# mikostrzewa/AprilSLAM

Hardware: AMD Instinct MI355X
Metric: frames/sec at 1280x720, 20 tags/frame (detection + batched PnP) (higher is better)
Workload: dtype u8/f64

## Files before the change

### aprilslam_amd/csrc/aprilslam.hip

```cpp
#include "../../include/aprilslam.h"

#include <algorithm>
#include <chrono>
#include <cmath>
#include <cstdarg>
#include <cstdio>
#include <cstring>
#include <memory>
#include <string>
#include <type_traits>
#include <vector>

#include "asl_common.h"
#include "tag_standard41h12.inc"
#include "k_wave.inc"

#include "k_threshold.inc"
#include "k_blur.inc"
#include "k_cc.inc"
#include "k_cluster.inc"
#include "k_seg.inc"
#include "k_quad.inc"
#include "k_decode.inc"
#include "k_pnp.inc"
// ... 472 lines not shown
    if (g.f == 2) {
        const unsigned int ntile = (unsigned int)(g.tw * g.th);
        const unsigned int nrest = (unsigned int)(g.sw - 4 * g.tw) * (unsigned int)g.sh + (unsigned int)(g.sh - 4 * g.th) * (unsigned int)(4 * g.tw);
        if (ntile)
            hipLaunchKernelGGL((g.channels == 1 ? k_decimate2_tiles<1> : k_decimate2_tiles<3>), dim3((ntile + 255) / 256, B), dim3(256), 0, st, d_frames, g,
                               d->dgray.p, d->tmin.p, d->tmax.p);
        if (nrest)
            hipLaunchKernelGGL((g.channels == 1 ? k_decimate_rest<1> : k_decimate_rest<3>), dim3((nrest + 255) / 256, B), dim3(256), 0, st, d_frames, g,
                               d->dgray.p);
    } else
        hipLaunchKernelGGL((g.channels == 1 ? k_decimate_minmax<1> : k_decimate_minmax<3>), dim3((g.sw + 63) / 64, (thx + 3) / 4, B), blk, 0, st, d_frames, g, d->dgray.p, d->tmin.p, d->tmax.p);

    d->qgray = d->dgray.p;
    if (d->blur.r) {
        STAGE("k_quad_blur");
        hipLaunchKernelGGL(k_quad_blur, dim3((g.sw + BLUR_TW - 1) / BLUR_TW, (g.sh + BLUR_TH - 1) / BLUR_TH, B), dim3(256), 0, st, d->dgray.p, g, d->blur,
                           d->bgray.p, d->tmin.p, d->tmax.p);
        d->qgray = d->bgray.p;
    }

    const int nwx = seg_nwx(g), pty = seg_point_tiles_y(g);
    const size_t nwords = (size_t)B * g.sh * nwx;
    STAGE("k_tile_cut");
    if (g.tw > 0 && g.th > 0)
        hipLaunchKernelGGL(k_tile_cut, dim3((((g.tw + 3) / 4) * ((g.th + 3) / 4) + 255) / 256, B), dim3(256), 0, st, d->tmin.p, d->tmax.p, g, d->tcut.p);
    STAGE("k_seg_tile");
    {
        const int ntiles = nwx * ((g.sh + SEG_TH - 1) / SEG_TH);
        hipLaunchKernelGGL(k_seg_tile, dim3((ntiles + SEG_TILE_WAVES - 1) / SEG_TILE_WAVES, 1, B), dim3(64 * SEG_TILE_WAVES), 0, st, d->qgray, d->tcut.p, g, nwx, ntiles,
                           d->wmask.p, d->bmask.p, d->parent.p, d->sizes.p, d->rootmask.p, d->seg_edges.p, d->dense_seg.p, d->counters.p);
        hipLaunchKernelGGL(k_seg_tile_dense, dim3(1024), dim3(64), 0, st, g, nwx, ntiles, d->wmask.p, d->bmask.p, d->parent.p, d->sizes.p,
                           d->rootmask.p, d->dense_seg.p, d->counters.p);
    }
    STAGE("k_seg_border");
    {
        const size_t nseams = nwx > 1 ? (size_t)B * g.sh * (nwx - 1) : 0;
        const unsigned int ncol_blocks = (unsigned int)((nseams + 63) / 64);
        const int nrb = (g.sh - 1) / SEG_TH;
        const unsigned int nrow_blocks = (unsigned int)nwx * (unsigned int)nrb * (unsigned int)B;
        if (ncol_blocks + nrow_blocks > 0)
            hipLaunchKernelGGL(k_seg_border, dim3(ncol_blocks + nrow_blocks), dim3(64), 0, st, d->wmask.p, d->bmask.p, d->seg_edges.p,
                               nwx * ((g.sh + SEG_TH - 1) / SEG_TH), g, nwx, d->parent.p, d->counters.p, ncol_blocks, nrb > 0 ? nrb : 1);
    }
    STAGE("k_seg_roots");
    hipLaunchKernelGGL(k_seg_roots, dim3((unsigned int)((nwords + 255) / 256)), dim3(256), 0, st, d->rootmask.p, g, nwx, d->parent.p, d->sizes.p);

    STAGE("k_seg_points");
    hipLaunchKernelGGL((k_seg_points<SEGP_PCAP, SEGP_RUNCAP, SEGP_NW, 1>), dim3(B, (nwx + SEGP_NW - 1) / SEGP_NW, pty), dim3(64 * SEGP_NW), 0, st,
                       d->wmask.p, d->bmask.p, g, nwx, d->parent.p, d->sizes.p, d->hkeys.p, d->hcounts.p, d->nslots - 1, d->stage_rec.p,
                       d->stage_pos.p, d->frame_cursor.p, d->stage_cap, d->dense_tiles.p, pty, d->counters.p);
    hipLaunchKernelGGL((k_seg_points<SEGP_PCAP_DENSE, SEGP_RUNCAP_DENSE, 1, 2>), dim3(256), dim3(64), 0, st, d->wmask.p, d->bmask.p, g, nwx,
                       d->parent.p, d->sizes.p, d->hkeys.p, d->hcounts.p, d->nslots - 1, d->stage_rec.p, d->stage_pos.p, d->frame_cursor.p,
                       d->stage_cap, d->dense_tiles.p, pty, d->counters.p);
    STAGE("k_cluster_filter");
    hipLaunchKernelGGL(k_cluster_filter, dim3((d->nslots + 1023) / 1024), dim3(1024), 0, st, d->hkeys.p, d->hcounts.p, d->nslots, g,
                       d->clusters.p, d->slot_cluster.p, d->class_lists.p, d->max_clusters, d->max_points, d->counters.p);
    STAGE("k_point_place");
    hipLaunchKernelGGL(k_point_place, dim3(16, B), dim3(256), 0, st, d->stage_rec.p, d->stage_pos.p, d->frame_cursor.p, d->stage_cap,
                       d->slot_cluster.p, d->points.p, d->counters.p);

    range_pop();
    range_push("S5 quad fit");
    for (int cls = 0; cls < NCLASSES; cls++) {
        static const char *const kFitStage[NCLASSES] = {"k_fit_quads<0>", "k_fit_quads<1>", "k_fit_quads<2>", "k_fit_quads<3>", "k_fit_quads<4>"};
        STAGE(kFitStage[cls]);
        launch_fit_class(d, g, cls, B, st);
    }

    STAGE("k_quad_finish");
    launch_quad_finish(d, g, st);
    range_pop();
    range_push("S6-S7 edge refinement, homography, decode");
    STAGE("k_quad_compact");
    hipLaunchKernelGGL(k_quad_compact, dim3((d->max_clusters + 1023) / 1024), dim3(1024), 0, st, d->quads.p, d->counters.p, d->max_clusters,
                       d->quad_list.p);
    unsigned int dgrid = std::min<unsigned int>(d->max_clusters, std::max<unsigned int>(8192u, 64u * B));
    STAGE("k_refine");
    hipLaunchKernelGGL((g.channels == 1 ? k_refine<1> : k_refine<3>), dim3(dgrid), dim3(64), 0, st, d->quads.p, d->counters.p, d->max_clusters, d_frames, g,
                       d->fam.reversed_border ? 1 : 0, d->refine, d->quadH.p, d->quad_list.p, d->side_mom.p);
    STAGE("k_homography");
    hipLaunchKernelGGL(k_homography, dim3(std::min<unsigned int>((d->max_clusters + 31) / 32, 2048u)), dim3(256), 0, st, d->quadH.p, d->counters.p, d->max_clusters,
                       d->quad_list.p, d->side_mom.p);
    STAGE("k_decode");
    hipLaunchKernelGGL((g.channels == 1 ? k_decode<1> : k_decode<3>), dim3(dgrid), dim3(64), 0, st, d->quads.p, d->quadH.p, d->counters.p, d->max_clusters, d_frames, g, d->fam,
                       d->maxhamming, d->dets.p, d->max_dets, d->counters.p, d->quad_list.p);

    range_pop();
    range_push("S9 PnP, S8 de-duplication");
    if (cam) {
        STAGE("k_pnp_dets");
        const int tpw = pnp_tpw(d->nd_guess ? d->nd_guess : (size_t)20 * B);
        hipLaunchKernelGGL(k_pnp_dets, dim3((d->max_dets + tpw - 1) / tpw), dim3(64), 0, st, d->dets.p, d->counters.p, d->max_dets, *cam, tpw);
    }
    STAGE("k_det_dedup");
    launch_dedup(S8Buffers{d->dets.p, d->counters.p, d->max_dets, d->frame_ndets.p, d->frame_idx.p, d->dets_per_frame, d->frame_nkeep.p, d->frame_off.p,
                           d->out_det.p, d->out_pose.p},
                 B, cam ? 1 : 0, st);
    range_pop();
    if (d->profiling && d->nev <= MAX_STAGES) HIPCHK(hipEventRecord(d->ev[d->nev], st));
    HIPCHK(hipGetLastError());
    return ASL_OK;
}

static CamDev make_cam(const asl_detector *d, const double *K, const double *dist, int n_dist, double tag_size)
{
    CamDev c;
    c.both_minima = d->pnp_both_minima; c.pad = 0;
    c.fx = K[0]; c.fy = K[4]; c.cx = K[2]; c.cy = K[5];
    c.k1 = c.k2 = c.p1 = c.p2 = c.k3 = 0;
    if (dist && n_dist >= 4) { c.k1 = dist[0]; c.k2 = dist[1]; c.p1 = dist[2]; c.p2 = dist[3]; }
    if (dist && n_dist >= 5) c.k3 = dist[4];
    c.half = (double)(float)(tag_size / 2);
    return c;
}

using clk = std::chrono::steady_clock;
static float msf(clk::time_point a, clk::time_point b) { return std::chrono::duration<float, std::milli>(b - a).count(); }

static int ensure_host_out(asl_detector *d, size_t want, size_t nframes)
{
    HIPCHK(d->host_nkeep.ensure(nframes, hipHostMallocDefault));
    if (want <= d->host_cap()) return ASL_OK;
    d->host_det.release(); d->host_pose.release();
    want = std::max<size_t>(want * 2, 4096);
    HIPCHK(d->host_det.ensure(want, hipHostMallocNonCoherent));
    HIPCHK(d->host_pose.ensure(want, hipHostMallocNonCoherent));
    return ASL_OK;
}

static int submit_batch(asl_detector *d, const uint8_t *d_frames, const Geom &g, hipStream_t st, const CamDev *cam)
{
    if (d->pending) return fail(ASL_EINVAL, "a batch is already in flight on this detector: collect it first");
    int rc = ensure_workspace(d, g);
    if (rc) return rc;
    d->t_submit = clk::now();
    rc = enqueue_detect(d, d_frames, g, st, cam);
    if (rc) return rc;
    HIPCHK(d->pinned_counters.ensure(CNT__N, hipHostMallocDefault));
    HIPCHK(hipMemcpyAsync(d->pinned_counters.p, d->counters.p, sizeof(long long) * CNT__N, hipMemcpyDeviceToHost, st));
    d->prefetched = 0;
    rc = ensure_host_out(d, std::min<size_t>(d->nd_guess, d->max_dets), (size_t)g.nframes);
    if (rc) return rc;
    HIPCHK(hipMemcpyAsync(d->host_nkeep.p, d->frame_nkeep.p, sizeof(unsigned int) * (size_t)g.nframes, hipMemcpyDeviceToHost, st));
    if (d->nd_guess > 0) {
        size_t guess = std::min<size_t>(d->nd_guess, d->max_dets);
        HIPCHK(hipMemcpyAsync(d->host_det.p, d->out_det.p, guess * sizeof(DetOut), hipMemcpyDeviceToHost, st));
        if (cam) HIPCHK(hipMemcpyAsync(d->host_pose.p, d->out_pose.p, guess * sizeof(PoseOut), hipMemcpyDeviceToHost, st));
        d->prefetched = guess;
    }
    d->pending = true;
    d->p_frames = d_frames; d->p_geom = g; d->p_stream = st; d->p_has_cam = cam != nullptr;
    if (cam) d->p_cam = *cam;
    d->t_enqueued = clk::now();
    return ASL_OK;
}

static int collect_batch(asl_detector *d, asl_detection *out, asl_pose *poses, int max_out, int *n_per_frame, int *n_out)
{
    if (!d->pending) return fail(ASL_EINVAL, "no batch in flight on this detector");
    const Geom g = d->p_geom;
    hipStream_t st = d->p_stream;
    const CamDev *cam = d->p_has_cam ? &d->p_cam : nullptr;
    clk::time_point t0 = d->t_submit, t1 = d->t_enqueued, t2 = t1;
    for (int attempt = 0; attempt < 4; attempt++) {
        if (attempt > 0) {
            d->pending = false;
            d->nd_guess = 0;
            int rc = submit_batch(d, d->p_frames, g, st, cam);
// ... 405 lines not shown
```

### aprilslam_amd/csrc/k_decode.inc

```

#define DEC_PROBE_GROUP 11
#define DEC_MAX_PROBES 44

__device__ __forceinline__ void half_angle_normal_dev(double a, double b, double *nx, double *ny)
{
    double r = sqrt(a * a + b * b);
    if (r == 0) { *nx = 1; *ny = 0; return; }
    double c2 = a / r;
    if (c2 >= 0) {
        double c = sqrt((1 + c2) / 2);
        *nx = c;
        *ny = b / (2 * r * c);
    } else {
        double s = sqrt((1 - c2) / 2);
        if (b < 0) s = -s;
        *ny = s;
        *nx = b / (2 * r * s);
    }
}

__device__ __forceinline__ double grp8_max(double v)
{
    v = fmax(v, dpp_mov<QUAD_XOR1>(0.0, v));
    v = fmax(v, dpp_mov<QUAD_XOR2>(0.0, v));
// ... 19 lines not shown
    const unsigned int nq = nq64 > (long long)max_clusters ? max_clusters : (unsigned int)nq64;
    const int lane = threadIdx.x & 63, r = lane & 7;
    for (unsigned int q0 = blockIdx.x * 32u; q0 < nq; q0 += gridDim.x * 32u) {
        const unsigned int qi = q0 + (threadIdx.x >> 3);
        const bool live = qi < nq;
        const unsigned int ci = quad_list[live ? qi : 0];
        double *const rec = corners_H + 10 * (size_t)ci;
        const double state = live ? rec[9] : 0.0;
        const bool todo = state == 0.5 || state == 0.25;
        const int e = r & 3;
        double Pex = todo ? rec[2 * e] : 0.0, Pey = todo ? rec[2 * e + 1] : 0.0;
        if (__any(state == 0.25)) {
            const double *in = edge_mom + ((size_t)(state == 0.25 ? ci : 0) * 4 + e) * 6;
            const double Mx = in[0], My = in[1], Mxx = in[2], Mxy = in[3], Myy = in[4], Nn = in[5];
            const double Ex = Mx / Nn, Ey = My / Nn;
            const double Cxx = Mxx / Nn - Ex * Ex, Cxy = Mxy / Nn - Ex * Ey, Cyy = Myy / Nn - Ey * Ey;
            double nx, ny;
            half_angle_normal_dev(Cyy - Cxx, -2 * Cxy, &nx, &ny);
            const double n0 = dpp_mov<QUAD_ROT1>(0.0, Ex), n1 = dpp_mov<QUAD_ROT1>(0.0, Ey), n2 = dpp_mov<QUAD_ROT1>(0.0, nx), n3 = dpp_mov<QUAD_ROT1>(0.0, ny);
            const double A00 = ny, A01 = -n3;
            const double A10 = -nx, A11 = n2;
            const double B0 = -Ex + n0;
            const double B1 = -Ey + n1;
            const double det = A00 * A11 - A10 * A01;
            const bool moved = fabs(det) > 0.001;
            const double W00 = A11 / det, W01 = -A01 / det;
            const double L0 = W00 * B0 + W01 * B1;
            const double cx = Ex + L0 * A00, cy = Ey + L0 * A10;
            const double fx = dpp_mov<QUAD_ROT3>(0.0, cx), fy = dpp_mov<QUAD_ROT3>(0.0, cy);
            const bool fm = dpp_mov<QUAD_ROT3>(0, moved ? 1 : 0) != 0;
            if (state == 0.25 && fm) { Pex = fx; Pey = fy; }
        }
        const int i = r >> 1;
        const double x = (i == 1 || i == 2) ? 1.0 : -1.0, y = (i >= 2) ? 1.0 : -1.0;
        const double u = __shfl(Pex, (lane & ~7) + i), v = __shfl(Pey, (lane & ~7) + i);
        double a[9];
        if ((r & 1) == 0) { a[0] = x; a[1] = y; a[2] = 1; a[3] = 0; a[4] = 0; a[5] = 0; a[6] = -x * u; a[7] = -y * u; a[8] = u; }
        else { a[0] = 0; a[1] = 0; a[2] = 0; a[3] = x; a[4] = y; a[5] = 1; a[6] = -x * v; a[7] = -y * v; a[8] = v; }
        int pos = r;
        bool ok = true;
#pragma unroll
        for (int col = 0; col < 8; col++) {
            const double val = pos >= col ? fabs(a[col]) : -1.0;
            const double mx = grp8_max(val);
            if (mx < 1e-10) ok = false;
            const int pivpos = grp8_min(val == mx ? pos : 99);
            const bool is_piv = pos == pivpos;
            if (is_piv) pos = col;
            else if (pos == col) pos = pivpos;
            const int src = grp8_owner(is_piv, lane);
            double piv[9];
#pragma unroll
            for (int j = col; j < 9; j++) piv[j] = __shfl(a[j], src);
            if (pos > col) {
                const double f = a[col] / piv[col];
                a[col] = 0.0;
#pragma unroll
                for (int j = col + 1; j < 9; j++) a[j] = a[j] - f * piv[j];
            }
        }
        double xs[8], mine = 0;
#pragma unroll
        for (int col = 7; col >= 0; col--) {
            double sum = 0;
#pragma unroll
            for (int k = col + 1; k < 8; k++) sum += a[k] * xs[k];
            const double xc = (a[8] - sum) / a[col];
            xs[col] = __shfl(xc, grp8_owner(pos == col, lane));
            if (r == col) mine = xs[col];
        }
        const bool all_ok = (__ballot(ok) >> (lane & ~7) & 0xFFull) == 0xFFull;
        if (todo) {
            rec[r] = mine;
            if (r == 0) { rec[8] = 1.0; rec[9] = all_ok ? 1.0 : 0.0; }
        }
    }
}

__device__ __forceinline__ void hproject_dev(const double *H, double x, double y, double *ox, double *oy)
{
    double xx = H[0] * x + H[1] * y + H[2];
    double yy = H[3] * x + H[4] * y + H[5];
    double zz = H[6] * x + H[7] * y + H[8];
    *ox = xx / zz;
    *oy = yy / zz;
}

struct GrayModel { double A[9], B[3], C[3]; };

__device__ __forceinline__ void gm_add_dev(GrayModel &gm, double x, double y, double gray)
{
    gm.A[0] += x * x; gm.A[1] += x * y; gm.A[2] += x; gm.A[4] += y * y; gm.A[5] += y; gm.A[8] += 1;
    gm.B[0] += x * gray; gm.B[1] += y * gray; gm.B[2] += gray;
}

__device__ __forceinline__ void gm_solve_dev(GrayModel &gm)
{
    const double *A = gm.A, *B = gm.B;
    double L[9], M[9], t[3];
    L[0] = sqrt(A[0]); L[3] = A[1] / L[0]; L[6] = A[2] / L[0];
    L[4] = sqrt(A[4] - L[3] * L[3]); L[7] = (A[5] - L[3] * L[6]) / L[4];
    L[8] = sqrt(A[8] - L[6] * L[6] - L[7] * L[7]);
    M[0] = 1 / L[0]; M[3] = -L[3] * M[0] / L[4]; M[4] = 1 / L[4];
    M[6] = (-L[6] * M[0] - L[7] * M[3]) / L[8]; M[7] = -L[7] * M[4] / L[8]; M[8] = 1 / L[8];
    t[0] = M[0] * B[0]; t[1] = M[3] * B[0] + M[4] * B[1]; t[2] = M[6] * B[0] + M[7] * B[1] + M[8] * B[2];
    gm.C[0] = M[0] * t[0] + M[3] * t[1] + M[6] * t[2];
    gm.C[1] = M[4] * t[1] + M[7] * t[2];
    gm.C[2] = M[8] * t[2];
}

__device__ __forceinline__ double gm_interp_dev(const GrayModel &gm, double x, double y) { return gm.C[0] * x + gm.C[1] * y + gm.C[2]; }

template <int CH>
__device__ __forceinline__ double value_for_pixel_dev(const uint8_t *frame, const Geom &g, double px, double py)
{
    int x1 = (int)floor(px - 0.5), x2 = (int)ceil(px - 0.5);
    double x = px - 0.5 - x1;
    int y1 = (int)floor(py - 0.5), y2 = (int)ceil(py - 0.5);
    double y = py - 0.5 - y1;
    if (x1 < 0 || x2 >= g.w || y1 < 0 || y2 >= g.h) return -1;
    return gray_at<CH>(frame, g, x1, y1) * (1 - x) * (1 - y) + gray_at<CH>(frame, g, x2, y1) * x * (1 - y) +
           gray_at<CH>(frame, g, x1, y2) * (1 - x) * y + gray_at<CH>(frame, g, x2, y2) * x * y;
}

__device__ __forceinline__ unsigned long long rotate90_dev(unsigned long long w, int nbits)
{
    int p = nbits;
    unsigned long long l = 0;
    if (nbits % 4 == 1) { p = nbits - 1; l = 1; }
    w = ((w >> l) << (p / 4 + l)) | (w >> (3 * p / 4 + l) << l) | (w & l);
    w &= ((1ull << nbits) - 1ull);
    return w;
}

#define PIX_EPS 9.5367431640625e-07

template <int CH>
__global__ void __launch_bounds__(64) k_refine(const QuadRec *__restrict__ quads, const long long *__restrict__ counters,
                                               unsigned int max_clusters, const uint8_t *__restrict__ frames, Geom g, int fam_reversed,
                                               int refine, double *__restrict__ Hout ,
                                               const unsigned int *__restrict__ quad_list, double *__restrict__ edge_mom )
{
    __shared__ double s_bx[64], s_by[64];
    __shared__ int s_bvalid[64];
    __shared__ double s_P[4][2];
    __shared__ int s_soff[5];
    __shared__ short s_probe[DEC_MAX_PROBES][64];
    __shared__ double s_enx[4], s_eny[4];
    int lane = threadIdx.x;
    PHASE_DECL();
    if (batch_poisoned(counters)) return;
    long long nq64 = counters[CNT_NQUADS];
    unsigned int nq = nq64 > (long long)max_clusters ? max_clusters : (unsigned int)nq64;

    for (unsigned int qi = blockIdx.x; qi < nq; qi += gridDim.x) {
        __syncthreads();
        PHASE_INIT();
        const unsigned int ci = quad_list[qi];
        const QuadRec *qp = quads + ci;
        const int q_valid = qp->valid, q_reversed = qp->reversed_border;
        if (lane == 0) Hout[10 * (size_t)ci + 9] = 0.0;
        if (!q_valid) continue;
        if (fam_reversed != q_reversed) continue;
        int fr = (int)(qp->key >> 48);
        const uint8_t *frame = frames + (size_t)fr * g.frame_pitch;
        if (lane < 4) {
            double px = qp->p[lane][0], py = qp->p[lane][1];
            if (g.f > 1) { px = (px - 0.5) * g.f + 0.5; py = (py - 0.5) * g.f + 0.5; }
// ... 73 lines not shown
                                }
                            }
                            at_prev = at[DEC_PROBE_GROUP - 1];
                        }
                    } else
                    for (int j0 = 0; j0 < nprobe; j0 += DEC_PROBE_GROUP) {
                        unsigned int raw[DEC_PROBE_GROUP], shv[DEC_PROBE_GROUP];
                        bool inside[DEC_PROBE_GROUP];
#pragma unroll
                        for (int u = 0; u < DEC_PROBE_GROUP; u++) {
                            double t = -(range + 1) + 0.25 * (j0 + u);
                            int xi = (int)(x0 + t * nx + PIX_EPS), yi = (int)(y0 + t * ny + PIX_EPS);
                            inside[u] = j0 + u < nprobe && (unsigned int)xi < (unsigned int)g.w && (unsigned int)yi < (unsigned int)g.h;
                            raw[u] = pixel_fetch<CH>(frame, g, inside[u] ? xi : 0, inside[u] ? yi : 0, &shv[u]);
                        }
#pragma unroll
                        for (int u = 0; u < DEC_PROBE_GROUP; u++)
                            if (j0 + u < nprobe) s_probe[j0 + u][lane] = inside[u] ? (short)pixel_gray<CH>(raw[u], shv[u]) : (short)-1;
                    }
                    PHASE(25);
                    int isum = 0, wsum = 0;
                    const int k0 = 4 * (g.f + 1);
                    for (int k = 0; k < steps; k++) {
                        const int g1 = s_probe[k + 8][lane], g2 = s_probe[k][lane];
                        const int dg = g2 - g1;
                        const int wgt = (g1 < 0 || g2 < 0 || g1 < g2) ? 0 : dg * dg;
                        isum += wgt * (k - k0);
                        wsum += wgt;
                    }
                    Mn = 0.25 * (double)isum;
                    Mcount = (double)wsum;
                } else {
                    for (int k = 0; k < steps; k++) {
                        double n = -range + 0.25 * k;
                        int x1 = (int)(x0 + (n + 1) * nx + PIX_EPS), y1 = (int)(y0 + (n + 1) * ny + PIX_EPS);
                        if (x1 < 0 || x1 >= g.w || y1 < 0 || y1 >= g.h) continue;
                        int x2 = (int)(x0 + (n - 1) * nx + PIX_EPS), y2 = (int)(y0 + (n - 1) * ny + PIX_EPS);
                        if (x2 < 0 || x2 >= g.w || y2 < 0 || y2 >= g.h) continue;
                        int g1 = gray_at<CH>(frame, g, x1, y1), g2 = gray_at<CH>(frame, g, x2, y2);
                        if (g1 < g2) continue;
                        double weight = (double)((g2 - g1) * (g2 - g1));
                        Mn += weight * n;
                        Mcount += weight;
                    }
                }
                if (Mcount == 0) { s_bvalid[lane] = 0; }
                else {
                    double n0 = Mn / Mcount;
                    s_bx[lane] = x0 + n0 * nx;
                    s_by[lane] = y0 + n0 * ny;
                    s_bvalid[lane] = 1;
                }
                }
            }
            __syncthreads();
            PHASE(26);
            if (lane < 4) {
                const int edge = lane;
                const int lo = (soff[edge] > base ? soff[edge] : base) - base;
                const int hi = (soff[edge + 1] < base + 64 ? soff[edge + 1] : base + 64) - base;
                for (int k = lo; k < hi; k++) {
                    if (!s_bvalid[k]) continue;
                    double bx = s_bx[k], by = s_by[k];
                    Mx += bx; My += by; Mxx += bx * bx; Mxy += bx * by; Myy += by * by; Nn++;
                }
            }
            __syncthreads();
            PHASE(27);
            }
            if (lane < 4) {
                double *out = edge_mom + ((size_t)ci * 4 + lane) * 6;
                out[0] = Mx; out[1] = My; out[2] = Mxx; out[3] = Mxy; out[4] = Myy; out[5] = Nn;
            }
        }

        PHASE(17);
        if (lane < 8) Hout[10 * (size_t)ci + lane] = s_P[lane >> 1][lane & 1];
        if (lane == 0) Hout[10 * (size_t)ci + 9] = refine ? 0.25 : 0.5;
        PHASE(22);
    }
    PHASE_FLUSH(16);
}

template <int CH>
__global__ void __launch_bounds__(64) __attribute__((amdgpu_waves_per_eu(5))) k_decode(const QuadRec *__restrict__ quads, const double *__restrict__ Hin,
                                               const long long *__restrict__ counters, unsigned int max_clusters,
                                               const uint8_t *__restrict__ frames, Geom g, FamilyDev fam, int maxhamming, DetRec *dets,
                                               unsigned int max_dets, long long *wcounters, const unsigned int *__restrict__ quad_list)
{
    __shared__ double s_H[9];
    __shared__ double s_smp[40][4];
    __shared__ double s_values[16 * 16], s_list[2 * 64];
    __shared__ double s_smpxy[40][2], s_bitxy[64][2];
    __shared__ GrayModel s_white, s_black;
    __shared__ int s_ok;
    int lane = threadIdx.x;
    PHASE_DECL();
    if (batch_poisoned(counters)) return;
    long long nq64 = counters[CNT_NQUADS];
    unsigned int nq = nq64 > (long long)max_clusters ? max_clusters : (unsigned int)nq64;

    {
        const int wb = fam.width_at_border;
        if (lane < 8 * wb && lane < 40) {
            int pi = lane / wb, i = lane % wb;
            double p0, p1, p2, p3;
            switch (pi) {
            case 0: p0 = -0.5; p1 = 0.5; p2 = 0; p3 = 1; break;
            case 1: p0 = 0.5; p1 = 0.5; p2 = 0; p3 = 1; break;
            case 2: p0 = wb + 0.5; p1 = .5; p2 = 0; p3 = 1; break;
            case 3: p0 = wb - 0.5; p1 = .5; p2 = 0; p3 = 1; break;
            case 4: p0 = 0.5; p1 = -0.5; p2 = 1; p3 = 0; break;
            case 5: p0 = 0.5; p1 = 0.5; p2 = 1; p3 = 0; break;
            case 6: p0 = 0.5; p1 = wb + 0.5; p2 = 1; p3 = 0; break;
            default: p0 = 0.5; p1 = wb - 0.5; p2 = 1; p3 = 0; break;
            }
            double tagx01 = (p0 + i * p2) / wb, tagy01 = (p1 + i * p3) / wb;
            s_smpxy[lane][0] = 2 * (tagx01 - 0.5);
            s_smpxy[lane][1] = 2 * (tagy01 - 0.5);
        }
        if (lane < fam.nbits) {
            int bitx = fam.bit_x[lane], bity = fam.bit_y[lane];
            double tagx01 = (bitx + 0.5) / wb, tagy01 = (bity + 0.5) / wb;
            s_bitxy[lane][0] = 2 * (tagx01 - 0.5);
            s_bitxy[lane][1] = 2 * (tagy01 - 0.5);
        }
    }
    for (unsigned int qi = blockIdx.x; qi < nq; qi += gridDim.x) {
        __syncthreads();
        PHASE_INIT();
        const unsigned int ci = quad_list[qi];
        if (Hin[10 * (size_t)ci + 9] == 0.0) continue;
        unsigned long long qkey = quads[ci].key;
        int fr = (int)(qkey >> 48);
        const uint8_t *frame = frames + (size_t)fr * g.frame_pitch;
        if (lane < 9) s_H[lane] = Hin[10 * (size_t)ci + lane];
        __syncthreads();
        int wb = fam.width_at_border, tw = fam.total_width;

        PHASE(18);
        int nsmp = 8 * wb;
        if (lane < nsmp && lane < 40) {
            const double tagx = s_smpxy[lane][0], tagy = s_smpxy[lane][1];
            double px, py;
            hproject_dev(s_H, tagx, tagy, &px, &py);
            int ix = (int)px, iy = (int)py;
            const bool inside = !(ix < 0 || iy < 0 || ix >= g.w || iy >= g.h);
            const double gv = (double)gray_at<CH>(frame, g, inside ? ix : 0, inside ? iy : 0);
            s_smp[lane][0] = inside ? tagx : 0.0; s_smp[lane][1] = inside ? tagy : 0.0; s_smp[lane][2] = inside ? gv : 0.0; s_smp[lane][3] = inside ? 1.0 : 0.0;
        }
        __syncthreads();
        {
            const int a = lane % 9, m = lane / 9;
            const int ku = a <= 2 ? 0 : (a <= 4 ? 1 : (a == 5 ? 3 : (a == 6 ? 0 : (a == 7 ? 1 : 2))));
            const int kv = a == 0 ? 0 : (a == 1 ? 1 : (a == 3 ? 1 : (a == 6 || a == 7 ? 2 : 3)));
            double acc = 0;
            if (lane < 18) {
                const int ns = nsmp < 40 ? nsmp : 40;
                for (int p0 = m * wb; p0 < ns; p0 += 2 * wb) {
                    const int pe = p0 + wb < ns ? p0 + wb : ns;
                    for (int smp = p0; smp < pe; smp++) {
                        const double u = s_smp[smp][ku], v = s_smp[smp][kv];
                        acc += u * v;
                    }
                }
            }
            GrayModel gm;
            const int base = (lane & 1) * 9;
            gm.A[0] = __shfl(acc, base + 0); gm.A[1] = __shfl(acc, base + 1); gm.A[2] = __shfl(acc, base + 2);
            gm.A[3] = 0; gm.A[4] = __shfl(acc, base + 3); gm.A[5] = __shfl(acc, base + 4);
            gm.A[6] = 0; gm.A[7] = 0; gm.A[8] = __shfl(acc, base + 5);
            gm.B[0] = __shfl(acc, base + 6); gm.B[1] = __shfl(acc, base + 7); gm.B[2] = __shfl(acc, base + 8);
            gm.C[0] = 0; gm.C[1] = 0; gm.C[2] = 0;
            gm_solve_dev(gm);
            if (lane == 0) s_white = gm;
            if (lane == 1) s_black = gm;
            const double at0 = gm_interp_dev(gm, 0, 0);
            const double w0 = __shfl(at0, 0), b0 = __shfl(at0, 1);
            if (lane == 0) {
                bool flip = (w0 - b0 < 0);
                s_ok = (flip == (fam.reversed_border != 0)) ? 1 : 0;
            }
        }
        for (int i = lane; i < tw * tw; i += 64) s_values[i] = 0;
        __syncthreads();
        if (!s_ok) continue;

        PHASE(19);
        int min_coord = (wb - tw) / 2;
        int bit_cell = 0, cell_x = 0, cell_y = 0;
        if (lane < fam.nbits) {
            int bitx = fam.bit_x[lane], bity = fam.bit_y[lane];
            cell_x = bitx - min_coord; cell_y = bity - min_coord;
            bit_cell = tw * cell_y + cell_x;
            const double tagx = s_bitxy[lane][0], tagy = s_bitxy[lane][1];
            double px, py;
            hproject_dev(s_H, tagx, tagy, &px, &py);
            double v = value_for_pixel_dev<CH>(frame, g, px, py);
            if (v != -1) {
                double thresh = (gm_interp_dev(s_black, tagx, tagy) + gm_interp_dev(s_white, tagx, tagy)) / 2.0;
                s_values[bit_cell] = v - thresh;
            }
        }
        __syncthreads();
        double sharp_v = 0.0;
        if (lane < fam.nbits) {
            double sv = 0;
            if (cell_y - 1 >= 0) sv += s_values[bit_cell - tw] * -1.0;
            if (cell_x - 1 >= 0) sv += s_values[bit_cell - 1] * -1.0;
            sv += s_values[bit_cell] * 4.0;
            if (cell_x + 1 <= tw - 1) sv += s_values[bit_cell + 1] * -1.0;
            if (cell_y + 1 <= tw - 1) sv += s_values[bit_cell + tw] * -1.0;
            sharp_v = s_values[bit_cell] + 0.25 * sv;
        }

        PHASE(20);
        float black_score, white_score, black_count, white_count;
        unsigned long long rcode;
        {
            const bool isbit = lane < fam.nbits;
            const double v = isbit ? sharp_v : 0.0;
            const bool isw = isbit && v > 0;
            const unsigned long long wm = __ballot(isw), bm = __ballot(isbit && !isw);
            rcode = __brevll(wm) >> (64 - fam.nbits);
            const unsigned long long below = (1ull << lane) - 1ull;
            if (isbit) s_list[isw ? __popcll(wm & below) : 64 + __popcll(bm & below)] = isw ? v : -v;
            __syncthreads();
            float score = 0;
            if (lane < 2) {
                const int cnt = lane == 0 ? __popcll(wm) : __popcll(bm);
                const double *list = s_list + 64 * lane;
                for (int k = 0; k < cnt; k++) score = (float)((double)score + list[k]);
            }
            white_score = __shfl(score, 0);
            black_score = __shfl(score, 1);
            white_count = (float)(1 + __popcll(wm));
            black_count = (float)(1 + __popcll(bm));
        }
        int id = -1, hamming = 255, rotation = 0;
        if (fam.idx_nch > 0) {
            unsigned int best = 0xFFFFFFFFu;
            const int ridx = lane >> 2, c = lane & 3;
            unsigned long long rr = rcode;
#pragma unroll
            for (int k = 1; k < 4; k++) {
                const unsigned long long t = rotate90_dev(rr, fam.nbits);
                rr = ridx >= k ? t : rr;
            }
            if (lane < 16 && c < fam.idx_nch) {
                const int lo = c == 0 ? fam.idx_lo[0] : (c == 1 ? fam.idx_lo[1] : (c == 2 ? fam.idx_lo[2] : fam.idx_lo[3]));
                const int w = c == 0 ? fam.idx_w[0] : (c == 1 ? fam.idx_w[1] : (c == 2 ? fam.idx_w[2] : fam.idx_w[3]));
                const unsigned int b = idx_bucket((rr >> lo) & ((1ull << w) - 1ull), w);
                const unsigned short *st = fam.idx_start + (size_t)c * (IDX_BUCKETS + 1) + b;
                const unsigned long long *ent = fam.idx_entries + (size_t)c * fam.ncodes;
                const unsigned int k1 = st[1];
                for (unsigned int k = st[0]; k < k1; k++) {
                    const unsigned long long en = ent[k];
                    const unsigned int dd = (unsigned int)__popcll(rr ^ (en & 0xFFFFFFFFFFFFull));
                    const unsigned int packed = ((unsigned int)ridx << 24) | (dd << 16) | (unsigned int)(en >> 48);
                    if (dd <= (unsigned int)maxhamming && packed < best) best = packed;
                }
            }
            best = wave_scan<true>(best, 0xFFFFFFFFu, [](unsigned int a, unsigned int b2) { return a < b2 ? a : b2; });
            if (best != 0xFFFFFFFFu) { id = (int)(best & 0xFFFFu); hamming = (int)((best >> 16) & 0xFFu); rotation = (int)(best >> 24); }
        } else {
            for (int ridx = 0; ridx < 4; ridx++) {
                unsigned int best = 0xFFFFFFFFu;
                for (int i = lane; i < fam.ncodes; i += 64) {
                    unsigned int dd = (unsigned int)__popcll(rcode ^ fam.codes[i]);
                    unsigned int packed = (dd << 16) | (unsigned int)i;
                    best = packed < best ? packed : best;
                }
                for (int off = 32; off > 0; off >>= 1) {
                    unsigned int o = (unsigned int)__shfl_xor((int)best, off);
                    best = o < best ? o : best;
                }
                if ((best >> 16) <= (unsigned int)maxhamming) { id = (int)(best & 0xFFFFu); hamming = (int)(best >> 16); rotation = ridx; break; }
                rcode = rotate90_dev(rcode, fam.nbits);
            }
        }
        PHASE(21);
        float margin = fminf(white_score / white_count, black_score / black_count);
        if (!(margin >= 0) || hamming >= 255) continue;

        if (lane == 0) {
            unsigned int di = (unsigned int)atomicAdd((unsigned long long *)&wcounters[CNT_NDETS], 1ull);
            if (di >= max_dets) { atomicAdd((unsigned long long *)&wcounters[CNT_OVERFLOW_DETS], 1ull); }
            else {
                const double C[4] = {1, 0, -1, 0}, Sn[4] = {0, 1, 0, -1};
                double c = C[rotation], s = Sn[rotation], Hr[9];
                for (int r = 0; r < 3; r++) {
                    Hr[3 * r + 0] = s_H[3 * r + 0] * c + s_H[3 * r + 1] * s;
                    Hr[3 * r + 1] = s_H[3 * r + 0] * -s + s_H[3 * r + 1] * c;
                    Hr[3 * r + 2] = s_H[3 * r + 2];
                }
                DetRec *d = &dets[di];
                d->id = id; d->hamming = hamming; d->margin = margin; d->frame = fr; d->key = qkey;
                d->pose_ok = 0; d->pad = 0;
                hproject_dev(Hr, 0, 0, &d->center[0], &d->center[1]);
                for (int i = 0; i < 4; i++) {
                    int tcx = (i == 1 || i == 2) ? 1 : -1, tcy = (i < 2) ? 1 : -1;
                    hproject_dev(Hr, tcx, tcy, &d->corners[i][0], &d->corners[i][1]);
                }
            }
        }
        PHASE(23);
    }
    PHASE_FLUSH(16);
}
```

### aprilslam_amd/csrc/k_wave.inc

```

#define QUAD_XOR1 0xB1
#define QUAD_XOR2 0x4E
#define QUAD_ROT1 0x39
#define QUAD_ROT2 0x4E
#define QUAD_ROT3 0x93

template <int CTRL, int ROWMASK = 0xf, int BANKMASK = 0xf, typename T>
__device__ __forceinline__ T dpp_mov(T old, T v)
{
    static_assert(sizeof(T) == 4 || sizeof(T) == 8, "32- or 64-bit values");
    if constexpr (sizeof(T) == 4) {
        return __builtin_bit_cast(T, __builtin_amdgcn_update_dpp(__builtin_bit_cast(int, old), __builtin_bit_cast(int, v), CTRL, ROWMASK, BANKMASK, false));
    } else {
        const unsigned long long ou = __builtin_bit_cast(unsigned long long, old), vu = __builtin_bit_cast(unsigned long long, v);
        const unsigned int lo = (unsigned int)__builtin_amdgcn_update_dpp((int)(unsigned int)ou, (int)(unsigned int)vu, CTRL, ROWMASK, BANKMASK, false);
        const unsigned int hi = (unsigned int)__builtin_amdgcn_update_dpp((int)(unsigned int)(ou >> 32), (int)(unsigned int)(vu >> 32), CTRL, ROWMASK, BANKMASK, false);
        return __builtin_bit_cast(T, ((unsigned long long)hi << 32) | lo);
    }
}

template <int K, typename T>
__device__ __forceinline__ T quad_bcast(T v)
{
    return dpp_mov<K * 0x55>(T(0), v);
}

template <typename T>
__device__ __forceinline__ T readlane(T v, int l)
{
    static_assert(sizeof(T) == 4 || sizeof(T) == 8, "32- or 64-bit values");
    if constexpr (sizeof(T) == 4) {
        return __builtin_bit_cast(T, __builtin_amdgcn_readlane(__builtin_bit_cast(int, v), l));
    } else {
        const unsigned long long vu = __builtin_bit_cast(unsigned long long, v);
        const unsigned int lo = (unsigned int)__builtin_amdgcn_readlane((int)(unsigned int)vu, l), hi = (unsigned int)__builtin_amdgcn_readlane((int)(unsigned int)(vu >> 32), l);
        return __builtin_bit_cast(T, ((unsigned long long)hi << 32) | lo);
    }
}

template <int J>
__device__ __forceinline__ unsigned int lane_xor32(unsigned int v)
{
    static_assert(J == 1 || J == 2 || J == 4 || J == 8 || J == 16 || J == 32, "power of two below 64");
    if constexpr (J == 1) return (unsigned int)__builtin_amdgcn_update_dpp(0, (int)v, 0xB1, 0xf, 0xf, false);
    else if constexpr (J == 2) return (unsigned int)__builtin_amdgcn_update_dpp(0, (int)v, 0x4E, 0xf, 0xf, false);
    else if constexpr (J == 4) {
        const int t = __builtin_amdgcn_update_dpp((int)v, (int)v, 0x104, 0xf, 0x5, false);
        return (unsigned int)__builtin_amdgcn_update_dpp(t, (int)v, 0x114, 0xf, 0xA, false);
    } else if constexpr (J == 8) return (unsigned int)__builtin_amdgcn_update_dpp(0, (int)v, 0x128, 0xf, 0xf, false);
    else if constexpr (J == 16) {
        const auto r = __builtin_amdgcn_permlane16_swap(v, v, false, false);
        return (__lane_id() & 16u) ? r[0] : r[1];
    } else {
        const auto r = __builtin_amdgcn_permlane32_swap(v, v, false, false);
        return (__lane_id() & 32u) ? r[0] : r[1];
    }
}

template <int J>
__device__ __forceinline__ unsigned long long lane_xor(unsigned long long v)
{
    return ((unsigned long long)lane_xor32<J>((unsigned int)(v >> 32)) << 32) | lane_xor32<J>((unsigned int)v);
}

template <bool REDUCE, typename T, typename Op>
__device__ __forceinline__ T wave_scan(T v, T ident, Op op)
{
    v = op(v, dpp_mov<0x111>(ident, v));
    v = op(v, dpp_mov<0x112>(ident, v));
    v = op(v, dpp_mov<0x114>(ident, v));
    v = op(v, dpp_mov<0x118>(ident, v));
    v = op(v, dpp_mov<0x142, 0xa>(ident, v));
    v = op(v, dpp_mov<0x143, 0xc>(ident, v));
    if constexpr (REDUCE) return readlane(v, 63);
    else return v;
}

template <int LANES, typename T>
__device__ __forceinline__ T butterfly_sum(T v)
{
    static_assert(LANES == 1 || LANES == 2 || LANES == 4 || LANES == 8 || LANES == 16 || LANES == 32 || LANES == 64, "power of two up to 64");
    static_assert(__is_same(T, double) || __is_same(T, int), "double or int");
    if constexpr (LANES > 1) {
        v = butterfly_sum<LANES / 2>(v);
        if constexpr (sizeof(T) == 8) v += __builtin_bit_cast(double, lane_xor<LANES / 2>(__builtin_bit_cast(unsigned long long, v)));
        else v += (int)lane_xor32<LANES / 2>((unsigned int)v);
    }
    return v;
}
```

Measured before the change: 389,700.

## Decode four quads per wavefront using 16-lane rows with dynamic LDS

Restructures k_decode so each 64-lane block handles four quads at once, one per 16-lane row. Per-quad shared state moves into a dynamically sized LDS region, and wave-wide reductions become row-local DPP reductions and broadcasts. Bit-grid cell coordinates are precomputed, and the final det write is spread across lanes. It also swaps the two divides in homography projection for a reciprocal helper. The aim is to stop wasting most of the lanes in a wave that only needed 9–40 active threads per quad, at the cost of more loops per lane and extra syncs.

After: 393,500 (median of 6 runs). No clear change (+1.0%).

```diff
diff --git a/aprilslam_amd/csrc/aprilslam.hip b/aprilslam_amd/csrc/aprilslam.hip
--- a/aprilslam_amd/csrc/aprilslam.hip
+++ b/aprilslam_amd/csrc/aprilslam.hip
@@ -578,8 +578,13 @@
     hipLaunchKernelGGL(k_homography, dim3(std::min<unsigned int>((d->max_clusters + 31) / 32, 2048u)), dim3(256), 0, st, d->quadH.p, d->counters.p, d->max_clusters,
                        d->quad_list.p, d->side_mom.p);
     STAGE("k_decode");
-    hipLaunchKernelGGL((g.channels == 1 ? k_decode<1> : k_decode<3>), dim3(dgrid), dim3(64), 0, st, d->quads.p, d->quadH.p, d->counters.p, d->max_clusters, d_frames, g, d->fam,
-                       d->maxhamming, d->dets.p, d->max_dets, d->counters.p, d->quad_list.p);
+    {
+        const unsigned int ngroups = (d->max_clusters + 3) / 4;
+        const unsigned int grid = std::min<unsigned int>(ngroups, std::max<unsigned int>(4096u, 8u * B));
+        const size_t lds = 4 * sizeof(double) * (size_t)decode_row_doubles(d->fam.nbits, d->fam.width_at_border, d->fam.total_width);
+        hipLaunchKernelGGL((g.channels == 1 ? k_decode<1> : k_decode<3>), dim3(grid), dim3(64), lds, st, d->quads.p, d->quadH.p, d->counters.p, d->max_clusters, d_frames, g,
+                           d->fam, d->maxhamming, d->dets.p, d->max_dets, d->counters.p, d->quad_list.p);
+    }
 
     range_pop();
     range_push("S9 PnP, S8 de-duplication");
diff --git a/aprilslam_amd/csrc/k_decode.inc b/aprilslam_amd/csrc/k_decode.inc
--- a/aprilslam_amd/csrc/k_decode.inc
+++ b/aprilslam_amd/csrc/k_decode.inc
@@ -125,8 +125,9 @@
     double xx = H[0] * x + H[1] * y + H[2];
     double yy = H[3] * x + H[4] * y + H[5];
     double zz = H[6] * x + H[7] * y + H[8];
-    *ox = xx / zz;
-    *oy = yy / zz;
+    const Recip k = recip_of(zz);
+    *ox = div_by(xx, k);
+    *oy = div_by(yy, k);
 }
 
 struct GrayModel { double A[9], B[3], C[3]; };
@@ -366,27 +367,38 @@
     PHASE_FLUSH(16);
 }
 
+#define DEC_ROW_HEAD 16
+__host__ __device__ __forceinline__ int decode_row_doubles(int nbits, int wb, int tw)
+{
+    const int ns = 8 * wb < 40 ? 8 * wb : 40;
+    const int smp = 4 * ns, grid = tw * tw + nbits;
+    return DEC_ROW_HEAD + (smp > grid ? smp : grid);
+}
+
 template <int CH>
 __global__ void __launch_bounds__(64) __attribute__((amdgpu_waves_per_eu(5))) k_decode(const QuadRec *__restrict__ quads, const double *__restrict__ Hin,
                                                const long long *__restrict__ counters, unsigned int max_clusters,
                                                const uint8_t *__restrict__ frames, Geom g, FamilyDev fam, int maxhamming, DetRec *dets,
                                                unsigned int max_dets, long long *wcounters, const unsigned int *__restrict__ quad_list)
 {
-    __shared__ double s_H[9];
-    __shared__ double s_smp[40][4];
-    __shared__ double s_values[16 * 16], s_list[2 * 64];
+    extern __shared__ double s_rows[];
     __shared__ double s_smpxy[40][2], s_bitxy[64][2];
-    __shared__ GrayModel s_white, s_black;
-    __shared__ int s_ok;
-    int lane = threadIdx.x;
+    __shared__ unsigned short s_bitcell[64];
+    const int lane = threadIdx.x, r = lane >> 4, j = lane & 15;
     PHASE_DECL();
     if (batch_poisoned(counters)) return;
     long long nq64 = counters[CNT_NQUADS];
     unsigned int nq = nq64 > (long long)max_clusters ? max_clusters : (unsigned int)nq64;
+    const int wb = fam.width_at_border, tw = fam.total_width, nbits = fam.nbits;
+    const int ns = 8 * wb < 40 ? 8 * wb : 40;
+    double *const s_H = s_rows + r * decode_row_doubles(nbits, wb, tw);
+    double *const s_C = s_H + 10;
+    double(*const s_smp)[4] = (double(*)[4])(s_H + DEC_ROW_HEAD);
+    double *const s_sums = s_H + DEC_ROW_HEAD;
+    double *const s_values = s_H + DEC_ROW_HEAD, *const s_list = s_values + tw * tw;
 
     {
-        const int wb = fam.width_at_border;
-        if (lane < 8 * wb && lane < 40) {
+        if (lane < ns) {
             int pi = lane / wb, i = lane % wb;
             double p0, p1, p2, p3;
             switch (pi) {
@@ -403,135 +415,144 @@
             s_smpxy[lane][0] = 2 * (tagx01 - 0.5);
             s_smpxy[lane][1] = 2 * (tagy01 - 0.5);
         }
-        if (lane < fam.nbits) {
+        if (lane < nbits) {
             int bitx = fam.bit_x[lane], bity = fam.bit_y[lane];
             double tagx01 = (bitx + 0.5) / wb, tagy01 = (bity + 0.5) / wb;
             s_bitxy[lane][0] = 2 * (tagx01 - 0.5);
             s_bitxy[lane][1] = 2 * (tagy01 - 0.5);
+            const int min_coord = (wb - tw) / 2;
+            s_bitcell[lane] = (unsigned short)(((bity - min_coord) << 8) | (bitx - min_coord));
         }
     }
-    for (unsigned int qi = blockIdx.x; qi < nq; qi += gridDim.x) {
+    for (unsigned int g0 = blockIdx.x * 4u; g0 < nq; g0 += gridDim.x * 4u) {
         __syncthreads();
         PHASE_INIT();
-        const unsigned int ci = quad_list[qi];
-        if (Hin[10 * (size_t)ci + 9] == 0.0) continue;
-        unsigned long long qkey = quads[ci].key;
-        int fr = (int)(qkey >> 48);
+        const unsigned int qi = g0 + r;
+        const unsigned int ci = quad_list[qi < nq ? qi : g0];
+        const double *const rec = Hin + 10 * (size_t)ci;
+        bool live = qi < nq && rec[9] != 0.0;
+        if (!__any(live)) continue;
+        const int fr = live ? (int)(quads[ci].key >> 48) : 0;
         const uint8_t *frame = frames + (size_t)fr * g.frame_pitch;
-        if (lane < 9) s_H[lane] = Hin[10 * (size_t)ci + lane];
-        __syncthreads();
-        int wb = fam.width_at_border, tw = fam.total_width;
+        if (j < 9) s_H[j] = live ? rec[j] : (j % 4 == 0 ? 1.0 : 0.0);
+        __syncthreads();
 
         PHASE(18);
-        int nsmp = 8 * wb;
-        if (lane < nsmp && lane < 40) {
-            const double tagx = s_smpxy[lane][0], tagy = s_smpxy[lane][1];
-            double px, py;
-            hproject_dev(s_H, tagx, tagy, &px, &py);
-            int ix = (int)px, iy = (int)py;
-            const bool inside = !(ix < 0 || iy < 0 || ix >= g.w || iy >= g.h);
-            const double gv = (double)gray_at<CH>(frame, g, inside ? ix : 0, inside ? iy : 0);
-            s_smp[lane][0] = inside ? tagx : 0.0; s_smp[lane][1] = inside ? tagy : 0.0; s_smp[lane][2] = inside ? gv : 0.0; s_smp[lane][3] = inside ? 1.0 : 0.0;
+        for (int s0 = 0; s0 < ns; s0 += 16) {
+            const int s = s0 + j;
+            if (s < ns) {
+                const double tagx = s_smpxy[s][0], tagy = s_smpxy[s][1];
+                double px, py;
+                hproject_dev(s_H, tagx, tagy, &px, &py);
+                int ix = (int)px, iy = (int)py;
+                const bool inside = !(ix < 0 || iy < 0 || ix >= g.w || iy >= g.h);
+                const double gv = (double)gray_at<CH>(frame, g, inside ? ix : 0, inside ? iy : 0);
+                s_smp[s][0] = inside ? tagx : 0.0; s_smp[s][1] = inside ? tagy : 0.0; s_smp[s][2] = inside ? gv : 0.0; s_smp[s][3] = inside ? 1.0 : 0.0;
+            }
         }
         __syncthreads();
         {
-            const int a = lane % 9, m = lane / 9;
+            const int a = j;
             const int ku = a <= 2 ? 0 : (a <= 4 ? 1 : (a == 5 ? 3 : (a == 6 ? 0 : (a == 7 ? 1 : 2))));
             const int kv = a == 0 ? 0 : (a == 1 ? 1 : (a == 3 ? 1 : (a == 6 || a == 7 ? 2 : 3)));
-            double acc = 0;
-            if (lane < 18) {
-                const int ns = nsmp < 40 ? nsmp : 40;
-                for (int p0 = m * wb; p0 < ns; p0 += 2 * wb) {
-                    const int pe = p0 + wb < ns ? p0 + wb : ns;
-                    for (int smp = p0; smp < pe; smp++) {
-                        const double u = s_smp[smp][ku], v = s_smp[smp][kv];
-                        acc += u * v;
+            double accw = 0, accb = 0;
+            if (a < 9) {
+                for (int p0 = 0; p0 < ns; p0 += 2 * wb) {
+                    for (int i = 0; i < wb; i++) {
+                        const int sw = p0 + i, sb = sw + wb;
+                        if (sw < ns) accw += s_smp[sw][ku] * s_smp[sw][kv];
+                        if (sb < ns) accb += s_smp[sb][ku] * s_smp[sb][kv];
                     }
                 }
             }
+            __syncthreads();
+            if (a < 9) { s_sums[a] = accw; s_sums[9 + a] = accb; }
+            __syncthreads();
             GrayModel gm;
-            const int base = (lane & 1) * 9;
-            gm.A[0] = __shfl(acc, base + 0); gm.A[1] = __shfl(acc, base + 1); gm.A[2] = __shfl(acc, base + 2);
-            gm.A[3] = 0; gm.A[4] = __shfl(acc, base + 3); gm.A[5] = __shfl(acc, base + 4);
-            gm.A[6] = 0; gm.A[7] = 0; gm.A[8] = __shfl(acc, base + 5);
-            gm.B[0] = __shfl(acc, base + 6); gm.B[1] = __shfl(acc, base + 7); gm.B[2] = __shfl(acc, base + 8);
+            const double *const sm = s_sums + (j & 1) * 9;
+            gm.A[0] = sm[0]; gm.A[1] = sm[1]; gm.A[2] = sm[2];
+            gm.A[3] = 0; gm.A[4] = sm[3]; gm.A[5] = sm[4];
+            gm.A[6] = 0; gm.A[7] = 0; gm.A[8] = sm[5];
+            gm.B[0] = sm[6]; gm.B[1] = sm[7]; gm.B[2] = sm[8];
             gm.C[0] = 0; gm.C[1] = 0; gm.C[2] = 0;
             gm_solve_dev(gm);
-            if (lane == 0) s_white = gm;
-            if (lane == 1) s_black = gm;
-            const double at0 = gm_interp_dev(gm, 0, 0);
-            const double w0 = __shfl(at0, 0), b0 = __shfl(at0, 1);
-            if (lane == 0) {
-                bool flip = (w0 - b0 < 0);
-                s_ok = (flip == (fam.reversed_border != 0)) ? 1 : 0;
-            }
-        }
-        for (int i = lane; i < tw * tw; i += 64) s_values[i] = 0;
-        __syncthreads();
-        if (!s_ok) continue;
+            if (j < 2) { s_C[3 * j + 0] = gm.C[0]; s_C[3 * j + 1] = gm.C[1]; s_C[3 * j + 2] = gm.C[2]; }
+            const double at0 = gm_interp_dev(gm, 0, 0), other = dpp_mov<QUAD_XOR1>(0.0, at0);
+            const double w0 = (j & 1) ? other : at0, b0 = (j & 1) ? at0 : other;
+            const bool flip = (w0 - b0 < 0);
+            live = live && (row_field(__ballot(flip == (fam.reversed_border != 0))) & 1u);
+        }
+        __syncthreads();
+        for (int i = j; i < tw * tw; i += 16) s_values[i] = 0;
+        __syncthreads();
+        if (!__any(live)) continue;
 
         PHASE(19);
-        int min_coord = (wb - tw) / 2;
-        int bit_cell = 0, cell_x = 0, cell_y = 0;
-        if (lane < fam.nbits) {
-            int bitx = fam.bit_x[lane], bity = fam.bit_y[lane];
-            cell_x = bitx - min_coord; cell_y = bity - min_coord;
-            bit_cell = tw * cell_y + cell_x;
-            const double tagx = s_bitxy[lane][0], tagy = s_bitxy[lane][1];
-            double px, py;
-            hproject_dev(s_H, tagx, tagy, &px, &py);
-            double v = value_for_pixel_dev<CH>(frame, g, px, py);
-            if (v != -1) {
-                double thresh = (gm_interp_dev(s_black, tagx, tagy) + gm_interp_dev(s_white, tagx, tagy)) / 2.0;
-                s_values[bit_cell] = v - thresh;
-            }
-        }
-        __syncthreads();
-        double sharp_v = 0.0;
-        if (lane < fam.nbits) {
-            double sv = 0;
-            if (cell_y - 1 >= 0) sv += s_values[bit_cell - tw] * -1.0;
-            if (cell_x - 1 >= 0) sv += s_values[bit_cell - 1] * -1.0;
-            sv += s_values[bit_cell] * 4.0;
-            if (cell_x + 1 <= tw - 1) sv += s_values[bit_cell + 1] * -1.0;
-            if (cell_y + 1 <= tw - 1) sv += s_values[bit_cell + tw] * -1.0;
-            sharp_v = s_values[bit_cell] + 0.25 * sv;
-        }
-
+        for (int b0 = 0; b0 < nbits; b0 += 16) {
+            const int b = b0 + j;
+            if (b < nbits && live) {
+                const int cell = s_bitcell[b];
+                const double tagx = s_bitxy[b][0], tagy = s_bitxy[b][1];
+                double px, py;
+                hproject_dev(s_H, tagx, tagy, &px, &py);
+                double v = value_for_pixel_dev<CH>(frame, g, px, py);
+                if (v != -1) {
+                    double thresh = ((s_C[3] * tagx + s_C[4] * tagy + s_C[5]) + (s_C[0] * tagx + s_C[1] * tagy + s_C[2])) / 2.0;
+                    s_values[tw * (cell >> 8) + (cell & 255)] = v - thresh;
+                }
+            }
+        }
+        __syncthreads();
+        unsigned long long white_bits = 0;
+        int wcnt = 0, bcnt = 0;
+        for (int b0 = 0; b0 < nbits; b0 += 16) {
+            const int b = b0 + j;
+            const bool isbit = b < nbits;
+            double v = 0.0;
+            if (isbit) {
+                const int cell = s_bitcell[b];
+                const int cell_x = cell & 255, cell_y = cell >> 8, bit_cell = tw * cell_y + cell_x;
+                double sv = 0;
+                if (cell_y - 1 >= 0) sv += s_values[bit_cell - tw] * -1.0;
+                if (cell_x - 1 >= 0) sv += s_values[bit_cell - 1] * -1.0;
+                sv += s_values[bit_cell] * 4.0;
+                if (cell_x + 1 <= tw - 1) sv += s_values[bit_cell + 1] * -1.0;
+                if (cell_y + 1 <= tw - 1) sv += s_values[bit_cell + tw] * -1.0;
+                v = s_values[bit_cell] + 0.25 * sv;
+            }
+            const bool isw = isbit && v > 0;
+            const unsigned int wf = row_field(__ballot(isw)), bf = row_field(__ballot(isbit && !isw));
+            const unsigned int below = (1u << j) - 1u;
+            if (isbit) s_list[isw ? wcnt + __popc(wf & below) : nbits - 1 - (bcnt + __popc(bf & below))] = isw ? v : -v;
+            wcnt += __popc(wf);
+            bcnt += __popc(bf);
+            white_bits |= (unsigned long long)wf << b0;
+        }
+        unsigned long long rcode = __brevll(white_bits) >> (64 - nbits);
+        __syncthreads();
         PHASE(20);
-        float black_score, white_score, black_count, white_count;
-        unsigned long long rcode;
+        float margin;
         {
-            const bool isbit = lane < fam.nbits;
-            const double v = isbit ? sharp_v : 0.0;
-            const bool isw = isbit && v > 0;
-            const unsigned long long wm = __ballot(isw), bm = __ballot(isbit && !isw);
-            rcode = __brevll(wm) >> (64 - fam.nbits);
-            const unsigned long long below = (1ull << lane) - 1ull;
-            if (isbit) s_list[isw ? __popcll(wm & below) : 64 + __popcll(bm & below)] = isw ? v : -v;
-            __syncthreads();
             float score = 0;
-            if (lane < 2) {
-                const int cnt = lane == 0 ? __popcll(wm) : __popcll(bm);
-                const double *list = s_list + 64 * lane;
-                for (int k = 0; k < cnt; k++) score = (float)((double)score + list[k]);
-            }
-            white_score = __shfl(score, 0);
-            black_score = __shfl(score, 1);
-            white_count = (float)(1 + __popcll(wm));
-            black_count = (float)(1 + __popcll(bm));
+            const int cnt = j == 0 ? wcnt : bcnt;
+            if (j < 2 && live) {
+                if (j == 0) for (int k = 0; k < cnt; k++) score = (float)((double)score + s_list[k]);
+                else for (int k = 0; k < cnt; k++) score = (float)((double)score + s_list[nbits - 1 - k]);
+            }
+            const float mean = score / (float)(1 + cnt);
+            margin = fminf(row_bcast(mean, 0), row_bcast(mean, 1));
         }
         int id = -1, hamming = 255, rotation = 0;
         if (fam.idx_nch > 0) {
             unsigned int best = 0xFFFFFFFFu;
-            const int ridx = lane >> 2, c = lane & 3;
+            const int ridx = j >> 2, c = j & 3;
             unsigned long long rr = rcode;
 #pragma unroll
             for (int k = 1; k < 4; k++) {
-                const unsigned long long t = rotate90_dev(rr, fam.nbits);
+                const unsigned long long t = rotate90_dev(rr, nbits);
                 rr = ridx >= k ? t : rr;
             }
-            if (lane < 16 && c < fam.idx_nch) {
+            if (live && c < fam.idx_nch) {
                 const int lo = c == 0 ? fam.idx_lo[0] : (c == 1 ? fam.idx_lo[1] : (c == 2 ? fam.idx_lo[2] : fam.idx_lo[3]));
                 const int w = c == 0 ? fam.idx_w[0] : (c == 1 ? fam.idx_w[1] : (c == 2 ? fam.idx_w[2] : fam.idx_w[3]));
                 const unsigned int b = idx_bucket((rr >> lo) & ((1ull << w) - 1ull), w);
@@ -545,47 +566,49 @@
                     if (dd <= (unsigned int)maxhamming && packed < best) best = packed;
                 }
             }
-            best = wave_scan<true>(best, 0xFFFFFFFFu, [](unsigned int a, unsigned int b2) { return a < b2 ? a : b2; });
+            best = row_min(best);
             if (best != 0xFFFFFFFFu) { id = (int)(best & 0xFFFFu); hamming = (int)((best >> 16) & 0xFFu); rotation = (int)(best >> 24); }
         } else {
+            bool found = false;
             for (int ridx = 0; ridx < 4; ridx++) {
                 unsigned int best = 0xFFFFFFFFu;
-                for (int i = lane; i < fam.ncodes; i += 64) {
+                for (int i = j; i < fam.ncodes; i += 16) {
                     unsigned int dd = (unsigned int)__popcll(rcode ^ fam.codes[i]);
                     unsigned int packed = (dd << 16) | (unsigned int)i;
                     best = packed < best ? packed : best;
                 }
-                for (int off = 32; off > 0; off >>= 1) {
-                    unsigned int o = (unsigned int)__shfl_xor((int)best, off);
-                    best = o < best ? o : best;
-                }
-                if ((best >> 16) <= (unsigned int)maxhamming) { id = (int)(best & 0xFFFFu); hamming = (int)(best >> 16); rotation = ridx; break; }
-                rcode = rotate90_dev(rcode, fam.nbits);
+                best = row_min(best);
+                if (!found && (best >> 16) <= (unsigned int)maxhamming) { id = (int)(best & 0xFFFFu); hamming = (int)(best >> 16); rotation = ridx; found = true; }
+                if (__all(found || !live)) break;
+                rcode = rotate90_dev(rcode, nbits);
             }
         }
         PHASE(21);
-        float margin = fminf(white_score / white_count, black_score / black_count);
-        if (!(margin >= 0) || hamming >= 255) continue;
-
-        if (lane == 0) {
-            unsigned int di = (unsigned int)atomicAdd((unsigned long long *)&wcounters[CNT_NDETS], 1ull);
-            if (di >= max_dets) { atomicAdd((unsigned long long *)&wcounters[CNT_OVERFLOW_DETS], 1ull); }
-            else {
-                const double C[4] = {1, 0, -1, 0}, Sn[4] = {0, 1, 0, -1};
-                double c = C[rotation], s = Sn[rotation], Hr[9];
-                for (int r = 0; r < 3; r++) {
-                    Hr[3 * r + 0] = s_H[3 * r + 0] * c + s_H[3 * r + 1] * s;
-                    Hr[3 * r + 1] = s_H[3 * r + 0] * -s + s_H[3 * r + 1] * c;
-                    Hr[3 * r + 2] = s_H[3 * r + 2];
-                }
-                DetRec *d = &dets[di];
-                d->id = id; d->hamming = hamming; d->margin = margin; d->frame = fr; d->key = qkey;
+        live = live && margin >= 0 && hamming < 255;
+        if (!__any(live)) continue;
+
+        unsigned int di = 0;
+        if (live && j == 0) di = (unsigned int)atomicAdd((unsigned long long *)&wcounters[CNT_NDETS], 1ull);
+        di = row_bcast(di, 0);
+        if (live && di >= max_dets) {
+            if (j == 0) atomicAdd((unsigned long long *)&wcounters[CNT_OVERFLOW_DETS], 1ull);
+        } else if (live && j < 5) {
+            const double c = rotation == 0 ? 1.0 : (rotation == 2 ? -1.0 : 0.0), s = rotation == 1 ? 1.0 : (rotation == 3 ? -1.0 : 0.0);
+            double Hr[9];
+#pragma unroll
+            for (int k = 0; k < 3; k++) {
+                Hr[3 * k + 0] = s_H[3 * k + 0] * c + s_H[3 * k + 1] * s;
+                Hr[3 * k + 1] = s_H[3 * k + 0] * -s + s_H[3 * k + 1] * c;
+                Hr[3 * k + 2] = s_H[3 * k + 2];
+            }
+            DetRec *d = &dets[di];
+            const int i = j - 1;
+            const int tcx = j == 0 ? 0 : ((i == 1 || i == 2) ? 1 : -1), tcy = j == 0 ? 0 : ((i < 2) ? 1 : -1);
+            double *const out = j == 0 ? d->center : d->corners[i];
+            hproject_dev(Hr, tcx, tcy, &out[0], &out[1]);
+            if (j == 0) {
+                d->id = id; d->hamming = hamming; d->margin = margin; d->frame = fr; d->key = quads[ci].key;
                 d->pose_ok = 0; d->pad = 0;
-                hproject_dev(Hr, 0, 0, &d->center[0], &d->center[1]);
-                for (int i = 0; i < 4; i++) {
-                    int tcx = (i == 1 || i == 2) ? 1 : -1, tcy = (i < 2) ? 1 : -1;
-                    hproject_dev(Hr, tcx, tcy, &d->corners[i][0], &d->corners[i][1]);
-                }
             }
         }
         PHASE(23);
diff --git a/aprilslam_amd/csrc/k_wave.inc b/aprilslam_amd/csrc/k_wave.inc
--- a/aprilslam_amd/csrc/k_wave.inc
+++ b/aprilslam_amd/csrc/k_wave.inc
@@ -88,3 +88,20 @@
     }
     return v;
 }
+
+__device__ __forceinline__ unsigned int row_min(unsigned int v)
+{
+    v = min(v, lane_xor32<1>(v));
+    v = min(v, lane_xor32<2>(v));
+    v = min(v, lane_xor32<4>(v));
+    return min(v, lane_xor32<8>(v));
+}
+template <typename T>
+__device__ __forceinline__ T row_bcast(T v, int k)
+{
+    return __shfl(v, (int)(__lane_id() & 48u) | k);
+}
+__device__ __forceinline__ unsigned int row_field(unsigned long long ballot)
+{
+    return (unsigned int)(ballot >> (__lane_id() & 48u)) & 0xFFFFu;
+}
```
